# allegro/allRank

Hardware: NVIDIA H100
Metric: slates/sec (higher is better)
Workload: dtype tf32

## Files before the change

### allrank_b200/csrc/gemm_tf32.h

```cpp
#pragma once
#include <cstdint>
#include <cuda_runtime.h>

#include "dropout.cuh"

namespace arb {

struct TRef {
  const void* ptr = nullptr;
  int64_t dim[4] = {1, 1, 1, 1};
  int64_t stride[4] = {1, 0, 0, 0};
  int bf16 = 0;
};

enum : int {
  EPI_BIAS = 1,
  EPI_RELU = 2,
  EPI_ADD_AUX = 4,
  EPI_MASK_AUX = 8,
  EPI_ATOMIC = 16,
  EPI_DROPOUT = 32,
  EPI_COLSUM = 64,
  EPI_RELU_BITS = 128,
  EPI_MASK_BITS = 256,
};

struct GemmDesc {
  int M = 0, N = 0, K = 0;
  int a_mn = 0, b_mn = 0;
  int b_tf32 = 0;
  int dgrad = 0;
  TRef A, B, C, Aux;
  int nb2 = 1, nb3 = 1;
  int a_b2 = 0, a_b3 = 0, b_b2 = 0, b_b3 = 0, c_b2 = 0, c_b3 = 0;
  int block_n = 64;
  int split_k = 1;
  int flags = 0;
  float alpha = 1.0f;
  const float* bias = nullptr;
  float* atomic_out = nullptr;
  int64_t atomic_ld = 0;
  DropSite drop{0u, 0u, 1.0f};
  float* colsum_out = nullptr;
  uint32_t* bits = nullptr;
  const int* rows_dev = nullptr;
};

int launch_gemm_tf32(const GemmDesc& d, cudaStream_t stream);

struct TmapBox { uint32_t b[4]; };
int make_tmap_4d(void* out_CUtensorMap, const TRef& t, TmapBox box, int unswizzled);

void set_tf32_round_on_load(int enable);
int tf32_round_on_load();
void set_gemm_persistent(int on);

}
```

### allrank_b200/csrc/scorer.cu

```cuda
#include <cstdint>
#include <string>
#include <vector>
#include <cuda_runtime.h>

#include "attention_fused.h"
#include "common.h"
#include "defaults.h"
#include "gemm_tf32.h"
#include "scorer_kernels.h"

namespace arb {

static inline int64_t align_up(int64_t v, int64_t a) { return (v + a - 1) / a * a; }

static int g_attn_mode = 2;
static int g_skip_padding = ARB_DEFAULT_SKIP_PADDING;
static int g_pack_rows = ARB_DEFAULT_PACK_ROWS;
static bool use_fused(const arb_scorer_config& c, int S) {
  return g_attn_mode >= 1 && c.n_layers > 0 && attn_fused_supported(S, c.d_model / c.n_heads);
}
static bool use_fused_bwd(const arb_scorer_config& c, int S) {
  return g_attn_mode >= 2 && use_fused(c, S) && attn_fused_bwd_supported(S, c.d_model / c.n_heads);
}

static inline int n_outputs(const arb_scorer_config& c) { return c.d_output > 1 ? c.d_output : 1; }

static int g_relu_bits = ARB_DEFAULT_RELU_BITS;
static bool relu_bits(const arb_scorer_config& c) {
  return g_relu_bits && c.n_layers > 0 && !c.bf16 && c.dropout == 0.0f && c.d_ff % 32 == 0;
}

static bool pack_eligible(const arb_scorer_config& c, int S) {
  return c.n_layers > 0 && use_fused_bwd(c, S) && c.dropout == 0.0f && c.fc_dropout == 0.0f && c.pe_mode == 0 &&
         n_outputs(c) == 1;
}
static bool use_pack(const arb_scorer_config& c, int S) { return g_pack_rows && g_skip_padding && pack_eligible(c, S); }

struct ParamLayout {
  int n_fc;
  int fc_size[ARB_MAX_FC_LAYERS];
  int64_t fc_w[ARB_MAX_FC_LAYERS], fc_b[ARB_MAX_FC_LAYERS];
  int64_t in_a, in_b;
  struct Layer { int64_t wqkv, bqkv, wo, bo, w1, b1, w2, b2, ln1_a, ln1_b, ln2_a, ln2_b; };
  Layer layer[64];
  int64_t lnf_a, lnf_b, head_w, head_b, pe, total;
};

static int make_param_layout(const arb_scorer_config& c, ParamLayout& L) {
  if (c.n_layers < 0 || c.n_layers > 64) { arb_set_error("scorer: n_layers must be in [0,64]"); return ARB_E_UNSUPPORTED; }
  if (c.d_model <= 0 || c.d_model % 4 || c.n_features <= 0 || c.n_features % 4) {
    arb_set_error("scorer: d_model and (padded) n_features must be positive multiples of 4");
    return ARB_E_UNSUPPORTED;
  }
  if (c.n_layers > 0) {
    if (c.n_heads <= 0 || c.d_model % c.n_heads || (c.d_model / c.n_heads) % 4 || c.d_ff <= 0 || c.d_ff % 4) {
      arb_set_error("scorer: need d_model % h == 0, (d_model/h) % 4 == 0 and d_ff % 4 == 0");
      return ARB_E_UNSUPPORTED;
    }
    if (c.d_model / c.n_heads > 128) { arb_set_error("scorer: head width above 128 is not supported"); return ARB_E_UNSUPPORTED; }
  }
  if (c.d_model > 1024) { arb_set_error("scorer: d_model above 1024 is not supported"); return ARB_E_UNSUPPORTED; }
  if (c.bf16 && c.n_layers > 0 && (c.d_model % 8 || c.d_ff % 8 || c.d_model < 64 || c.d_ff < 64)) {
    arb_set_error("scorer: bf16 mode needs d_model and d_ff to be multiples of 8, at least 64");
    return ARB_E_UNSUPPORTED;
  }
  const int64_t d = c.d_model, F = c.n_features, f = c.d_ff;
  L.n_fc = c.n_fc_layers > 0 ? c.n_fc_layers : 1;
  if (L.n_fc > ARB_MAX_FC_LAYERS) { arb_set_error("scorer: at most 8 FC layers"); return ARB_E_UNSUPPORTED; }
  for (int i = 0; i < L.n_fc; ++i) {
    L.fc_size[i] = c.n_fc_layers > 0 ? c.fc_sizes[i] : c.d_model;
    if (L.fc_size[i] <= 0 || L.fc_size[i] % 4 || L.fc_size[i] > 8192) {
      arb_set_error("scorer: FC layer widths must be positive multiples of 4, at most 8192");
      return ARB_E_UNSUPPORTED;
    }
  }
  if (L.fc_size[L.n_fc - 1] != c.d_model) { arb_set_error("scorer: the last FC width must equal d_model"); return ARB_E_INVALID_ARG; }
  if (c.fc_act < ARB_ACT_NONE || c.fc_act > ARB_ACT_RELU) { arb_set_error("scorer: unknown FC activation"); return ARB_E_UNSUPPORTED; }
  if (c.fc_input_norm && F > 1024) { arb_set_error("scorer: input_norm supports up to 1024 features"); return ARB_E_UNSUPPORTED; }
  int64_t o = 0;
  for (int i = 0; i < L.n_fc; ++i) {
    const int64_t in = i == 0 ? F : L.fc_size[i - 1];
    L.fc_w[i] = o; o += int64_t(L.fc_size[i]) * in;
// ... 384 lines not shown
    if (!indices || !table) { arb_set_error("scorer: positional encoding needs indices and a table"); return ARB_E_INVALID_ARG; }
    ARB_TRY(pos_forward(xcur, reinterpret_cast<const long long*>(indices), mask, table, c.pe_rows, sqrtf(float(d)), k.R, d, st));
  }
  if (pack) {
    ZeroRegions z;
    for (int l = 0; l < c.n_layers; ++l) {
      if (l > 0 && !training) break;
      const auto& wl = W.layer[l];
      if (!z.add(ws + wl.ctx, bf ? d / 2 : d, bf ? d / 2 : d, 1, 0)) {
        ARB_TRY(zero_rows(z, plan, k.R, st));
        z = ZeroRegions{};
        z.add(ws + wl.ctx, bf ? d / 2 : d, bf ? d / 2 : d, 1, 0);
      }
    }
    if (z.count) ARB_TRY(zero_rows(z, plan, k.R, st));
  }
  const AttnGeom geom{B, S, h, dk, k.R, poff};
  for (int l = 0; l < c.n_layers; ++l) {
    const auto& pl = L.layer[l];
    const auto& wl = W.layer[l];
    float* xn1 = ws + wl.xn1; float* qkv = ws + wl.qkv; float* prob = ws + wl.prob; float* ctx = ws + wl.ctx;
    float* xmid = ws + wl.xmid; float* xn2 = ws + wl.xn2; float* hdn = ws + wl.hdn; float* xout = ws + wl.xout;
    ARB_TRY(ln_forward(xcur, P + pl.ln1_a, P + pl.ln1_b, c.ln_eps, k.R, d, xn1, ws + wl.mean1, ws + wl.std1, st, 0,
                       bf ? xn1 : nullptr, plan));
    ARB_TRY(linear_fwd(k, act(xn1), d, d, wt(pl.wqkv), P + pl.bqkv, 3 * d, qkv, 3 * d, 0, nullptr, 0));
    if (W.fused) {
      ARB_TRY(launch_attn_fwd(attn_fwd_args(geom, qkv, act(ctx), mask, g_skip_padding ? kext : nullptr, ws + wl.smax,
                                            ws + wl.ssum, make_drop_site(seed, l, SITE_ATTN_P, p_drop)), st));
    } else {
      {
        GemmDesc g;
        g.M = S; g.N = S; g.K = dk; g.alpha = 1.0f / sqrtf(float(dk));
        g.A = head_view(qkv, dk, S, h, B, 3 * d);
        g.B = head_view(qkv + d, dk, S, h, B, 3 * d);
        g.C = prob_view(prob, S, W.Sp, h, B);
        batch_all(g, h, B); g.block_n = 64;
        ARB_TRY(launch_gemm_tf32(g, st));
      }
      ARB_TRY(softmax_forward(prob, mask, B, h, S, W.Sp, st, make_drop_site(seed, l, SITE_ATTN_P, p_drop)));
      {
        GemmDesc g;
        g.M = S; g.N = dk; g.K = S; g.b_mn = 1;
        g.A = prob_view(prob, S, W.Sp, h, B);
        g.B = head_view(qkv + 2 * d, dk, S, h, B, 3 * d);
        g.C = head_view(ctx, dk, S, h, B, d);
        batch_all(g, h, B); g.block_n = pick_block_n(dk);
        ARB_TRY(launch_gemm_tf32(g, st));
      }
    }
    ARB_TRY(linear_fwd(k, act(ctx), d, d, wt(pl.wo), P + pl.bo, d, xmid, d, EPI_ADD_AUX, xcur, d,
                       make_drop_site(seed, l, SITE_ATTN_OUT, p_drop)));
    ARB_TRY(ln_forward(xmid, P + pl.ln2_a, P + pl.ln2_b, c.ln_eps, k.R, d, xn2, ws + wl.mean2, ws + wl.std2, st, 0,
                       bf ? xn2 : nullptr, plan));
    ARB_TRY(linear_fwd(k, act(xn2), d, d, wt(pl.w1), P + pl.b1, f, act(hdn), f, EPI_RELU, nullptr, 0,
                       make_drop_site(seed, l, SITE_FFN_HID, p_drop),
                       wl.hbits ? reinterpret_cast<uint32_t*>(ws + wl.hbits) : nullptr));
    ARB_TRY(linear_fwd(k, act(hdn), f, f, wt(pl.w2), P + pl.b2, d, xout, d, EPI_ADD_AUX, xmid, d,
                       make_drop_site(seed, l, SITE_FFN_OUT, p_drop)));
    xcur = xout;
  }
  const int has_norm = c.n_layers > 0;
  if (hidden) {
    if (has_norm)
      return ln_forward(xcur, P + L.lnf_a, P + L.lnf_b, c.ln_eps, k.R, d, hidden, ws + W.meanf, ws + W.stdf, st, 0,
                        nullptr, plan, rowmap);
    if (cudaMemcpyAsync(hidden, xcur, size_t(k.R) * d * sizeof(float), cudaMemcpyDeviceToDevice, st) != cudaSuccess) {
      arb_set_error("scorer: device copy failed"); return ARB_E_CUDA;
    }
    return ARB_OK;
  }
  if (n_outputs(c) > 1) {
    const float* xf = xcur;
    if (has_norm) {
      ARB_TRY(ln_forward(xcur, P + L.lnf_a, P + L.lnf_b, c.ln_eps, k.R, d, ws + W.xf, ws + W.meanf, ws + W.stdf, st));
      xf = ws + W.xf;
    }
    return head_multi_forward(xf, P + L.head_w, P + L.head_b, c.out_act, k.R, d, n_outputs(c), scores, st);
  }
  ARB_TRY(head_forward(xcur, has_norm ? P + L.lnf_a : nullptr, has_norm ? P + L.lnf_b : nullptr, c.ln_eps, P + L.head_w,
                       P + L.head_b, has_norm, c.out_act, k.R, d, scores, ws + W.meanf, ws + W.stdf, st, plan, rowmap));
  return ARB_OK;
}

struct ScratchLayout { int64_t dxa, dxb, dxn, dxm, dqkv, dctx, dprob, prob, delta, dfa, dfb, ext, dy16, dxin, total; };
static void make_scratch_layout(const arb_scorer_config& c, const ParamLayout& L, int B, int S, ScratchLayout& Z,
                                bool want_dx = false) {
  const int64_t R = buffer_rows(c, B, S), d = c.d_model;
  const int Sp = int(align_up(S, 4));
  int64_t o = 0;
  auto take = [&](int64_t n) { int64_t at = o; o += align_up(n, 64); return at; };
  Z.dxa = take(R * d); Z.dxb = take(R * d); Z.dxn = take(R * d);
  Z.dxm = (c.dropout > 0.0f || c.fc_dropout > 0.0f || c.pe_mode != 0) ? take(R * d) : 0;
  if (c.n_layers > 0) {
    Z.dqkv = take(R * 3 * d); Z.dctx = take(R * d);
    const bool fb = use_fused_bwd(c, S);
    Z.dprob = fb ? 0 : take(int64_t(B) * c.n_heads * S * Sp);
    Z.prob = (use_fused(c, S) && !fb) ? take(int64_t(B) * c.n_heads * S * Sp) : 0;
    Z.delta = fb ? take(int64_t(B) * c.n_heads * S) : 0;
  } else {
    Z.dqkv = Z.dctx = Z.dprob = Z.prob = Z.delta = 0;
  }
  int64_t widest = c.fc_input_norm ? c.n_features : 0;
  for (int i = 0; i + 1 < L.n_fc; ++i) widest = std::max<int64_t>(widest, L.fc_size[i]);
  if (c.fc_act != ARB_ACT_NONE) widest = std::max<int64_t>(widest, d);
  Z.dfa = widest ? take(R * widest) : 0;
  Z.dfb = widest ? take(R * widest) : 0;
  Z.ext = take(B);
  Z.dy16 = (c.bf16 && c.n_layers > 0) ? take(R * d / 2) : 0;
  Z.dxin = (want_dx && pack_eligible(c, S)) ? take(R * c.n_features) : 0;
  Z.total = o;
}
// ... 45 lines not shown
  int* gext = reinterpret_cast<int*>(scratch + Z.ext);
  const bool skip = g_skip_padding && c.n_layers > 0 && use_fused_bwd(c, S);
  const bool pack = use_pack(c, S);
  const int* plan = pack ? reinterpret_cast<const int*>(ws + W.plan) : nullptr;
  const int* rowmap = pack ? reinterpret_cast<const int*>(ws + W.rowmap) : nullptr;
  const int* poff = pack ? reinterpret_cast<const int*>(ws + W.poff) : nullptr;
  if (pack) { k.rows_dev = plan; k.R = buffer_rows(c, B, S); x = ws + W.xc; gext = reinterpret_cast<int*>(ws + W.kext); }
  else if (skip) ARB_TRY(slate_extents(mask, dhidden ? dhidden : dscores, dhidden ? d : n_outputs(c), B, S, gext, st));
  const AttnGeom geom{B, S, h, dk, k.R, poff};
  if (pack) {
    ZeroRegions z;
    z.add(dctx, d, d, 0, 256);
    z.add(dqkv, bf ? 3 * d / 2 : 3 * d, bf ? 3 * d / 2 : 3 * d, 1, 0);
    ARB_TRY(zero_rows(z, plan, k.R, st));
  }
  const int has_norm = c.n_layers > 0;
  const float* xlast = c.n_layers > 0 ? ws + W.layer[c.n_layers - 1].xout : ws + W.x0;
  float* top_bias_grad = c.n_layers > 0 ? g(L.layer[c.n_layers - 1].b2) : fc_bias_grad;
  const float* dy = top_site.thresh ? dxm : dx;
  if (dhidden) {
    if (has_norm) {
      ARB_TRY(ln_backward(dhidden, xlast, P + L.lnf_a, ws + W.meanf, ws + W.stdf, c.ln_eps, nullptr, k.R, d, dx,
                          g(L.lnf_a), g(L.lnf_b), st, dxm, top_site, top_bias_grad, 0, nullptr, dy16, plan, rowmap));
    } else if (!fc_act) {
      if (fc_site.thresh || fc_bias_grad)
        ARB_TRY(act_backward(dhidden, ws + W.x0, dx, k.R, d, ARB_ACT_NONE, fc_site, 1.0f, fc_bias_grad, st));
      dy = (fc_site.thresh || fc_bias_grad) ? dx : dhidden;
    }
  } else if (n_outputs(c) > 1) {
    if (has_norm) {
      ARB_TRY(head_multi_backward(dscores, scores, ws + W.xf, P + L.head_w, c.out_act, k.R, d, n_outputs(c), dxn,
                                  g(L.head_w), g(L.head_b), st));
      ARB_TRY(ln_backward(dxn, xlast, P + L.lnf_a, ws + W.meanf, ws + W.stdf, c.ln_eps, nullptr, k.R, d, dx,
                          g(L.lnf_a), g(L.lnf_b), st, dxm, top_site, top_bias_grad, 0, nullptr, dy16));
    } else {
      ARB_TRY(head_multi_backward(dscores, scores, xlast, P + L.head_w, c.out_act, k.R, d, n_outputs(c), dx,
                                  g(L.head_w), g(L.head_b), st, dxm, top_site, top_bias_grad));
    }
  } else {
    ARB_TRY(head_backward(dscores, scores, xlast, has_norm ? P + L.lnf_a : nullptr, has_norm ? P + L.lnf_b : nullptr,
                          ws + W.meanf, ws + W.stdf, c.ln_eps, P + L.head_w, P + L.head_b, has_norm, c.out_act, k.R, d,
                          dx, has_norm ? g(L.lnf_a) : nullptr, has_norm ? g(L.lnf_b) : nullptr, g(L.head_w),
                          g(L.head_b), st, dxm, top_site, top_bias_grad, dy16, plan, rowmap));
  }
  for (int l = c.n_layers - 1; l >= 0; --l) {
    const auto& pl = L.layer[l];
    const auto& wl = W.layer[l];
    const float* xin = (l == 0) ? ws + W.x0 : ws + W.layer[l - 1].xout;
    float* xn1 = ws + wl.xn1; float* qkv = ws + wl.qkv; float* ctx = ws + wl.ctx;
    float* prob = W.fused ? scratch + Z.prob : ws + wl.prob;
    float* xmid = ws + wl.xmid; float* xn2 = ws + wl.xn2; float* hdn = ws + wl.hdn;
    const V dyv = bf ? b16(dy16) : V(dy);
    if (G) ARB_TRY(linear_bwd_weight(k, dyv, d, d, act(hdn), f, f, G + pl.w2));
    if (wl.hbits)
      ARB_TRY(linear_bwd_input(k, dyv, d, d, wt(pl.w2), f, act(hdn), f, EPI_COLSUM, nullptr, 0, 1.0f, g(pl.b1),
                               reinterpret_cast<const uint32_t*>(ws + wl.hbits)));
    else
    ARB_TRY(linear_bwd_input(k, dyv, d, d, wt(pl.w2), f, act(hdn), f, EPI_MASK_AUX | EPI_COLSUM, act(hdn), f,
                             drop_on ? 1.0f / (1.0f - p_drop) : 1.0f, g(pl.b1)));
    if (G) ARB_TRY(linear_bwd_weight(k, act(hdn), f, f, act(xn2), d, d, G + pl.w1));
    ARB_TRY(linear_bwd_input(k, act(hdn), f, f, wt(pl.w1), d, act(dxn), d, 0, nullptr, 0));
    const DropSite site_ao = make_drop_site(seed, l, SITE_ATTN_OUT, p_drop);
    ARB_TRY(ln_backward(dxn, xmid, P + pl.ln2_a, ws + wl.mean2, ws + wl.std2, c.ln_eps, dx, k.R, d, dx_alt,
                        g(pl.ln2_a), g(pl.ln2_b), st, dxm, site_ao, g(pl.bo), 0, bf ? dxn : nullptr, dy16, plan));
    dy = site_ao.thresh ? dxm : dx_alt;
    const V dyo = bf ? b16(dy16) : V(dy);
    if (G) ARB_TRY(linear_bwd_weight(k, dyo, d, d, act(ctx), d, d, G + pl.wo));
    ARB_TRY(linear_bwd_input(k, dyo, d, d, wt(pl.wo), d, dctx, d, 0, nullptr, 0));
    if (use_fused_bwd(c, S)) {
      ARB_TRY(launch_attn_bwd(attn_bwd_args(geom, qkv, act(ctx), dctx, dqkv, mask, (skip || pack) ? gext : nullptr,
                                            ws + wl.smax, ws + wl.ssum, scratch + Z.delta, g(pl.bqkv),
                                            make_drop_site(seed, l, SITE_ATTN_P, p_drop), plan, rowmap), st));
    } else {
      const DropSite site_p = make_drop_site(seed, l, SITE_ATTN_P, p_drop);
      if (W.fused || site_p.thresh) {
        GemmDesc g;
        g.M = S; g.N = S; g.K = dk; g.alpha = alpha;
        g.A = head_view(qkv, dk, S, h, B, 3 * d);
        g.B = head_view(qkv + d, dk, S, h, B, 3 * d);
        g.C = prob_view(prob, S, W.Sp, h, B);
        batch_all(g, h, B); g.block_n = 64;
        ARB_TRY(launch_gemm_tf32(g, st));
        ARB_TRY(softmax_forward(prob, mask, B, h, S, W.Sp, st));
      }
      {
        GemmDesc g;
        g.M = S; g.N = S; g.K = dk;
        g.A = head_view(dctx, dk, S, h, B, d);
        g.B = head_view(qkv + 2 * d, dk, S, h, B, 3 * d);
        g.C = prob_view(dprob, S, W.Sp, h, B);
        batch_all(g, h, B); g.block_n = 64;
        ARB_TRY(launch_gemm_tf32(g, st));
      }
      ARB_TRY(softmax_backward(dprob, prob, int64_t(B) * h * S, S, W.Sp, st, site_p));
      {
        GemmDesc g;
        g.M = S; g.N = dk; g.K = S; g.a_mn = 1; g.b_mn = 1;
        g.A = prob_view(prob, S, W.Sp, h, B);
        g.B = head_view(dctx, dk, S, h, B, d);
        g.C = head_view(dqkv + 2 * d, dk, S, h, B, 3 * d);
        batch_all(g, h, B); g.block_n = pick_block_n(dk);
        ARB_TRY(launch_gemm_tf32(g, st));
      }
      {
        GemmDesc g;
        g.M = S; g.N = dk; g.K = S; g.b_mn = 1; g.alpha = alpha;
        g.A = prob_view(dprob, S, W.Sp, h, B);
        g.B = head_view(qkv + d, dk, S, h, B, 3 * d);
        g.C = head_view(dqkv, dk, S, h, B, 3 * d);
        batch_all(g, h, B); g.block_n = pick_block_n(dk);
        ARB_TRY(launch_gemm_tf32(g, st));
      }
      {
        GemmDesc g;
// ... 247 lines not shown
```

### include/allrank_b200.h

```cpp
#ifndef ALLRANK_B200_H
#define ALLRANK_B200_H

#include <stddef.h>
#include <stdint.h>

#ifdef __cplusplus
extern "C" {
#endif

#define ARB_OK 0
#define ARB_E_INVALID_ARG (-1)
#define ARB_E_UNSUPPORTED (-2)
#define ARB_E_CUDA (-3)
#define ARB_E_WORKSPACE (-4)

#define ARB_MAX_ATS 32

#define ARB_SCHEME_NONE 0
#define ARB_SCHEME_NDCGLOSS1 1
#define ARB_SCHEME_NDCGLOSS2 2
#define ARB_SCHEME_LAMBDARANK 3
#define ARB_SCHEME_NDCGLOSS2PP 4
#define ARB_SCHEME_RANKNET 5
#define ARB_SCHEME_RANKNET_GTDIFF 6
// ... 98 lines not shown
                               const int64_t* indices, int32_t B, int32_t S, const float* scores,
                               const float* d_scores, const float* d_hidden, float* grads, float* d_x,
                               float* workspace, int64_t workspace_floats, float* scratch, int64_t scratch_floats,
                               uint64_t seed, void* stream);

int32_t arb_scorer_forward_dseed(const arb_scorer_config* cfg, const float* params, const float* x, const uint8_t* mask,
                                 const int64_t* indices, const float* pe_table,
                                 int32_t B, int32_t S, float* scores, float* workspace, int64_t workspace_floats,
                                 int32_t training, const uint64_t* seed_dev, void* stream);
int32_t arb_scorer_encode_dseed(const arb_scorer_config* cfg, const float* params, const float* x, const uint8_t* mask,
                                const int64_t* indices, const float* pe_table,
                                int32_t B, int32_t S, float* hidden, float* workspace, int64_t workspace_floats,
                                int32_t training, const uint64_t* seed_dev, void* stream);
int32_t arb_scorer_backward_ex_dseed(const arb_scorer_config* cfg, const float* params, const float* x,
                                     const uint8_t* mask, const int64_t* indices, int32_t B, int32_t S,
                                     const float* scores, const float* d_scores, const float* d_hidden, float* grads,
                                     float* d_x, float* workspace, int64_t workspace_floats, float* scratch,
                                     int64_t scratch_floats, const uint64_t* seed_dev, void* stream);

void arb_set_attention_mode(int32_t mode);

void arb_set_attention_skip_padding(int32_t on);

void arb_set_pack_rows(int32_t on);

void arb_set_attention_bwd_persistent(int32_t on);
int32_t arb_get_pack_rows(void);

void arb_set_pdl(int32_t on);

void arb_set_attention_fwd_two_pass(int32_t on);

void arb_set_gemm_persistent(int32_t on);

void arb_set_tf32_round_on_load(int32_t enable);

int32_t arb_gemm_tf32(const float* A, const float* B, float* C, const float* aux, const float* bias, int32_t M,
                      int32_t N, int32_t K, int32_t a_mn, int32_t b_mn, int32_t batch, int64_t a_bstride,
                      int64_t b_bstride, int64_t c_bstride, int32_t block_n, int32_t flags, float alpha,
                      int32_t split_k, void* stream);

int32_t arb_gemm_bf16(const void* A, const void* B, void* C, const void* aux, const float* bias, int32_t M, int32_t N,
                      int32_t K, int32_t a_mn, int32_t b_mn, int32_t block_n, int32_t flags, float alpha,
                      int32_t split_k, int32_t out_bf16, float* colsum_out, void* stream);

int32_t arb_attention_forward(const float* qkv, const uint8_t* mask, const int32_t* extent, int32_t B, int32_t S,
                              int32_t h, int32_t dk, float p, uint64_t seed, int32_t layer, int32_t ctx_bf16,
                              void* ctx, float* stat_max, float* stat_sum, void* stream);
int32_t arb_attention_backward(const float* qkv, const void* ctx, int32_t ctx_bf16, const float* d_ctx,
                               const uint8_t* mask, const int32_t* extent, const float* stat_max,
                               const float* stat_sum, int32_t B, int32_t S, int32_t h, int32_t dk, float p,
                               uint64_t seed, int32_t layer, void* d_qkv, float* dbias_qkv, float* delta_scratch,
                               void* stream);

int32_t arb_layernorm_forward(const float* x, const float* a, const float* b, float eps, int32_t torch_mode,
                              int64_t rows, int32_t width, float* y, void* y16, float* mean, float* sd,
                              const int32_t* rows_dev, const int32_t* rowmap, void* stream);
int32_t arb_layernorm_backward(const float* dy, const void* dy16_in, const float* x, const float* a, const float* mean,
                               const float* sd, float eps, int32_t torch_mode, const float* dres, int64_t rows,
                               int32_t width, float* dx, float* grad_a, float* grad_b, float* dx_masked,
                               void* dy16_out, float* colsum_out, float p, uint64_t seed, int32_t layer, int32_t site,
                               const int32_t* rows_dev, const int32_t* rowmap, void* stream);
int32_t arb_head_forward(const float* x, const float* a, const float* b, float eps, const float* w, const float* wb,
                         int32_t has_norm, int32_t act, int64_t rows, int32_t width, float* score, float* mean,
                         float* sd, const int32_t* rows_dev, const int32_t* rowmap, void* stream);
int32_t arb_head_backward(const float* dscore, const float* score, const float* x, const float* a, const float* b,
                          const float* mean, const float* sd, float eps, const float* w, int32_t has_norm, int32_t act,
                          int64_t rows, int32_t width, float* dx, float* grad_a, float* grad_b, float* grad_w,
                          float* grad_wb, float* dx_masked, void* dy16_out, float* colsum_out, float p, uint64_t seed,
                          int32_t layer, int32_t site, const int32_t* rows_dev, const int32_t* rowmap, void* stream);
int32_t arb_head_multi_forward(const float* xf, const float* w, const float* wb, int32_t act, int64_t rows,
                               int32_t width, int32_t n, float* score, void* stream);
int32_t arb_head_multi_backward(const float* dscore, const float* score, const float* xf, const float* w, int32_t act,
                                int64_t rows, int32_t width, int32_t n, float* dxf, float* grad_w, float* grad_wb,
                                float* dx_masked, float* colsum_out, float p, uint64_t seed, int32_t layer,
                                int32_t site, void* stream);
int32_t arb_column_sums(const float* in, int64_t rows, int32_t width, int64_t ld, float* out, void* stream);
int32_t arb_softmax_forward(float* scores, const uint8_t* mask, int32_t B, int32_t h, int32_t S, int32_t pitch,
                            float p, uint64_t seed, int32_t layer, void* stream);
int32_t arb_softmax_backward(float* dprob, float* prob, int64_t rows, int32_t S, int32_t pitch, float p,
                             uint64_t seed, int32_t layer, void* stream);

int32_t arb_adam_step(float* params, const float* grads, float* exp_avg, float* exp_avg_sq, int64_t n, float lr,
                      float beta1, float beta2, float eps, float weight_decay, int32_t step, float grad_scale,
                      void* stream);
int32_t arb_adam_step_dev(float* params, const float* grads, float* exp_avg, float* exp_avg_sq, int64_t n, float lr,
                          float beta1, float beta2, float eps, float weight_decay, float* state, float grad_scale,
                          void* stream);

size_t arb_assemble_slates_smem_bytes(int32_t max_query_len, int32_t S);
int32_t arb_assemble_slates(const float* docs_x, const float* docs_y, const int64_t* offsets, int64_t n_queries,
                            const int64_t* queries, int32_t B, int32_t S, int32_t F, int32_t max_query_len,
                            uint64_t seed, float* x_out, float* y_out, int64_t* idx_out, void* stream);
int32_t arb_gather_slates(const float* x, const float* y, const int32_t* order, int32_t B, int32_t S, int32_t F,
                          float* x_out, float* y_out, void* stream);

#define ARB_CLICK_MAX_NODES 32
#define ARB_CLICK_MAX_SLATE 4096
#define ARB_CLICK_FIXED 0
#define ARB_CLICK_RANDOM 1
#define ARB_CLICK_RELEVANT 2
#define ARB_CLICK_CASCADE 3
#define ARB_CLICK_MULTIPLE 4
#define ARB_CLICK_CONDITIONED 5
#define ARB_CLICK_MAXCLICKS 6
#define ARB_CLICK_DUPLICATES 7
// ... 30 lines not shown
```

Baseline: 196,800.

## Fuse FFN two-GEMM chain into one warp-specialized WGMMA kernel for forward and backward

Adds a persistent, warp-specialized TMA/WGMMA kernel that computes relu(x·W1+b1)·W2+b2+residual per 128-row tile, keeping the hidden chunk in shared memory. The backward path applies the same chaining to the input gradient, using the stored relu bitmask and emitting the b1 column sums. The aim is to avoid writing and re-reading the full d_ff hidden activation between the two GEMMs and to save kernel launches. In training the hidden tensor is still written for weight gradients. It only engages for d_model<=128 with enough rows, and it depends on pre-transposed weight buffers (wt32/wt32t) existing in the workspace.

```diff
diff --git a/allrank_b200/csrc/ffn_chain.cu b/allrank_b200/csrc/ffn_chain.cu
--- /dev/null
+++ b/allrank_b200/csrc/ffn_chain.cu
@@ -0,0 +1,415 @@
+#include <algorithm>
+#include <cstdio>
+#include <cuda.h>
+#include <cuda_runtime.h>
+
+#include "common.h"
+#include "gemm_tf32.h"
+#include "sm90_ptx.cuh"
+
+namespace arb {
+
+namespace {
+
+constexpr int CH_ROWS = 128;
+constexpr int CH_UNITS = 64;
+constexpr int UNIT_BYTES = 64 * 128;
+constexpr int X_SLAB_BYTES = CH_ROWS * 128;
+constexpr int H_SLAB_BYTES = 64 * 128;
+constexpr int CH_THREADS = 384;
+constexpr int SMEM_LIMIT = 227 * 1024;
+
+template <int D>
+struct ChainLayout {
+  static constexpr int KB1 = D / 32;
+  static constexpr int NBU = (D + 63) / 64;
+  static constexpr int X_BYTES = KB1 * X_SLAB_BYTES;
+  static constexpr int H_BYTES = 2 * 2 * H_SLAB_BYTES;
+  static constexpr int TAIL_BYTES = 1024;
+  static constexpr int NU_FIT = (SMEM_LIMIT - 1024 - TAIL_BYTES - X_BYTES - H_BYTES) / UNIT_BYTES;
+  static constexpr int NU = NU_FIT < 16 ? NU_FIT : 16;
+  static constexpr int RING_OFF = X_BYTES + H_BYTES;
+  static constexpr int TAIL_OFF = RING_OFF + NU * UNIT_BYTES;
+  static constexpr int total() { return TAIL_OFF + TAIL_BYTES + 1024; }
+  static_assert(D % 32 == 0 && D >= 32 && D <= 256, "d: a multiple of 32 up to 256");
+  static_assert(NU >= 2 * NBU, "the ring holds at least one k-block of the second product");
+  static_assert(total() <= SMEM_LIMIT, "shared memory budget");
+};
+
+struct ChainParams {
+  int M;
+  int F;
+  int rnd;
+  int store_h;
+  const float* b1;
+  const float* b2;
+  const float* aux;
+  float* y;
+  uint32_t* bits;
+  float* colsum;
+  const int* rows_dev;
+};
+
+__device__ __forceinline__ void load_a(uint32_t (&a)[4][4], const uint8_t* slab, int r0, int rnd) {
+  const int lane = threadIdx.x & 31, j = lane >> 3;
+#pragma unroll
+  for (int ks = 0; ks < 4; ++ks) {
+    ptx::ldmatrix_x4(a[ks], slab + ptx::sw128(r0 + 8 * (j & 1) + (lane & 7), 32 * ks + 16 * (j >> 1)));
+    if (rnd) {
+#pragma unroll
+      for (int e = 0; e < 4; ++e) a[ks][e] = ptx::cvt_tf32(__uint_as_float(a[ks][e]));
+    }
+  }
+}
+
+template <int D, int U = 0>
+__device__ __forceinline__ void second_mma(float (&acc)[D / 8][4], const uint32_t (&a)[4],
+                                           const uint64_t (&desc)[(D + 63) / 64], int ks) {
+  constexpr int WN = D % 64 == 0 ? 64 : 32;
+  if constexpr (U < D / WN) {
+    if constexpr (WN == 64) ptx::wgmma_m64n64k8_tf32<8 * U>(acc, a, desc[U] + 2 * ks);
+    else ptx::wgmma_m64n32k8_tf32<4 * U>(acc, a, desc[U / 2] + (U & 1) * (32 * 128 / 16) + 2 * ks);
+    second_mma<D, U + 1>(acc, a, desc, ks);
+  }
+}
+
+template <int D, bool BWD>
+__global__ void __launch_bounds__(CH_THREADS, 1) ffn_chain_kernel(const __grid_constant__ CUtensorMap tmX,
+                                                                 const __grid_constant__ CUtensorMap tmA,
+                                                                 const __grid_constant__ CUtensorMap tmB,
+                                                                 const __grid_constant__ CUtensorMap tmH,
+                                                                 const ChainParams p) {
+  using L = ChainLayout<D>;
+  constexpr int NU = L::NU, KB1 = L::KB1, NBU = L::NBU, NTY = D / 8;
+  extern __shared__ uint8_t smem_dyn[];
+  uint8_t* smem = reinterpret_cast<uint8_t*>((reinterpret_cast<uintptr_t>(smem_dyn) + 1023) & ~uintptr_t(1023));
+  uint8_t* xs = smem;
+  uint8_t* ring = smem + L::RING_OFF;
+  uint64_t* full = reinterpret_cast<uint64_t*>(smem + L::TAIL_OFF);
+  uint64_t* empty = full + NU;
+  uint64_t* xfull = empty + NU;
+  uint64_t* xfree = xfull + 8;
+  uint64_t* csfull = xfree + 1;
+  uint64_t* csempty = csfull + 2;
+  float* csx = reinterpret_cast<float*>(smem + L::TAIL_OFF + 512);
+
+  const int warp = threadIdx.x >> 5, lane = threadIdx.x & 31;
+  if (threadIdx.x == 0) {
+    ptx::prefetch_tmap(&tmX);
+    ptx::prefetch_tmap(&tmA);
+    ptx::prefetch_tmap(&tmB);
+    if (p.store_h) ptx::prefetch_tmap(&tmH);
+    for (int s = 0; s < NU; ++s) { ptx::mbar_init(&full[s], 1); ptx::mbar_init(&empty[s], 8); }
+    for (int kb = 0; kb < KB1; ++kb) ptx::mbar_init(&xfull[kb], 1);
+    ptx::mbar_init(xfree, 8);
+    for (int b = 0; b < 2; ++b) { ptx::mbar_init(&csfull[b], 128); ptx::mbar_init(&csempty[b], 128); }
+    ptx::fence_barrier_init();
+  }
+  arb_pdl_wait();
+  __syncthreads();
+  int n_tiles = (p.M + CH_ROWS - 1) / CH_ROWS;
+  if (p.rows_dev) n_tiles = min(n_tiles, (__ldg(p.rows_dev) + CH_ROWS - 1) / CH_ROWS);
+  const int n_chunks = p.F / CH_UNITS;
+
+  if (warp >= 8) {
+    asm volatile("setmaxnreg.dec.sync.aligned.u32 40;" ::: "memory");
+    if (warp == 8 && lane == 0) {
+      uint32_t it = 0;
+      auto unit = [&](const CUtensorMap* tm, int c0, int c1) {
+        const int s = it % NU;
+        const uint32_t round = it / NU;
+        if (round > 0) ptx::mbar_wait(&empty[s], (round - 1) & 1);
+        ptx::mbar_expect_tx(&full[s], UNIT_BYTES);
+        ptx::tma_load_4d(ring + s * UNIT_BYTES, tm, &full[s], c0, c1, 0, 0);
+        ++it;
+      };
+      int local = 0;
+      for (int t = blockIdx.x; t < n_tiles; t += gridDim.x, ++local) {
+        const int m0 = t * CH_ROWS;
+        if (local > 0) ptx::mbar_wait(xfree, (local - 1) & 1);
+        for (int kb = 0; kb < KB1; ++kb) {
+          ptx::mbar_expect_tx(&xfull[kb], X_SLAB_BYTES);
+          ptx::tma_load_4d(xs + kb * X_SLAB_BYTES, &tmX, &xfull[kb], 32 * kb, m0, 0, 0);
+        }
+        if (!BWD) {
+          const long long bytes = (long long)(min(p.M, m0 + CH_ROWS) - m0) * D * 4;
+          asm volatile("cp.async.bulk.prefetch.L2.global [%0], %1;"
+                       ::"l"(p.aux + (long long)m0 * D), "r"(uint32_t(bytes)) : "memory");
+        }
+        for (int j = 0; j < n_chunks; ++j) {
+          for (int kb = 0; kb < KB1; ++kb) unit(&tmA, 32 * kb, CH_UNITS * j);
+          for (int kb2 = 0; kb2 < 2; ++kb2)
+            for (int u = 0; u < NBU; ++u) unit(&tmB, CH_UNITS * j + 32 * kb2, 64 * u);
+        }
+      }
+    }
+  } else {
+    asm volatile("setmaxnreg.inc.sync.aligned.u32 232;" ::: "memory");
+    const int g = warp >> 2, w = warp & 3, gq = lane >> 2, t4 = lane & 3, gt = threadIdx.x & 127;
+    uint8_t* hs = smem + L::X_BYTES + g * 2 * H_SLAB_BYTES;
+    const int fw = p.F >> 5;
+    uint32_t it = 0, cj = 0;
+    int local = 0;
+    for (int t = blockIdx.x; t < n_tiles; t += gridDim.x, ++local) {
+      const int m0 = t * CH_ROWS;
+      const int row0 = m0 + 64 * g + 16 * w + gq;
+      float accY[NTY][4];
+#pragma unroll
+      for (int n = 0; n < NTY; ++n) accY[n][0] = accY[n][1] = accY[n][2] = accY[n][3] = 0.f;
+#pragma unroll 1
+      for (int j = 0; j < n_chunks; ++j, ++cj) {
+        uint32_t mw[2][2] = {{0u, 0u}, {0u, 0u}};
+        if constexpr (BWD) {
+#pragma unroll
+          for (int h = 0; h < 2; ++h)
+            if (row0 + 8 * h < p.M) {
+              mw[h][0] = __ldg(p.bits + (long long)(row0 + 8 * h) * fw + 2 * j);
+              mw[h][1] = __ldg(p.bits + (long long)(row0 + 8 * h) * fw + 2 * j + 1);
+            }
+        }
+        float accH[8][4];
+#pragma unroll
+        for (int n = 0; n < 8; ++n) accH[n][0] = accH[n][1] = accH[n][2] = accH[n][3] = 0.f;
+#pragma unroll 1
+        for (int kb = 0; kb < KB1; ++kb, ++it) {
+          const int s = it % NU;
+          ptx::mbar_wait(&full[s], (it / NU) & 1);
+          if (j == 0) ptx::mbar_wait(&xfull[kb], local & 1);
+          uint32_t a[4][4];
+          load_a(a, xs + kb * X_SLAB_BYTES, 64 * g + 16 * w, p.rnd);
+          const uint64_t desc = ptx::wgmma_desc_sw128(ring + s * UNIT_BYTES);
+          ptx::wgmma_fence_acc(accH);
+          ptx::wgmma_fence();
+#pragma unroll
+          for (int ks = 0; ks < 4; ++ks) ptx::wgmma_m64n64k8_tf32<0>(accH, a[ks], desc + 2 * ks);
+          ptx::wgmma_commit();
+          ptx::wgmma_wait0();
+          ptx::wgmma_fence_acc(accH);
+          __syncwarp();
+          if (lane == 0) ptx::mbar_arrive(&empty[s]);
+        }
+        if (j == n_chunks - 1) {
+          __syncwarp();
+          if (lane == 0) ptx::mbar_arrive(xfree);
+        }
+        if (p.store_h && lane == 0) ptx::tma_store_wait_read<0>();
+        if (BWD && p.colsum) ptx::named_bar_sync(1 + g, 128);
+        __syncwarp();
+        uint32_t wb[2][2] = {{0u, 0u}, {0u, 0u}};
+#pragma unroll
+        for (int n = 0; n < 8; ++n) {
+          const int c = 8 * n + 2 * t4, bp = 8 * (n & 3) + 2 * t4;
+          float2 bb = make_float2(0.f, 0.f);
+          if constexpr (!BWD) bb = __ldg(reinterpret_cast<const float2*>(p.b1 + CH_UNITS * j + c));
+#pragma unroll
+          for (int h = 0; h < 2; ++h) {
+            float o0 = accH[n][2 * h], o1 = accH[n][2 * h + 1];
+            if constexpr (BWD) {
+              o0 = (mw[h][n >> 2] >> bp) & 1u ? o0 : 0.f;
+              o1 = (mw[h][n >> 2] >> (bp + 1)) & 1u ? o1 : 0.f;
+            } else {
+              o0 += bb.x; o1 += bb.y;
+              o0 = fmaxf(o0, 0.0f); o1 = fmaxf(o1, 0.0f);
+              wb[h][n >> 2] |= (o0 > 0.f ? 1u : 0u) << bp | (o1 > 0.f ? 1u : 0u) << (bp + 1);
+            }
+            *reinterpret_cast<float2*>(hs + (n >> 2) * H_SLAB_BYTES + ptx::sw128(16 * w + gq + 8 * h, 4 * (c & 31))) =
+                make_float2(o0, o1);
+          }
+        }
+        if (!BWD && p.bits) {
+#pragma unroll
+          for (int h = 0; h < 2; ++h)
+#pragma unroll
+            for (int s = 0; s < 2; ++s) {
+              wb[h][s] |= __shfl_xor_sync(0xffffffffu, wb[h][s], 1);
+              wb[h][s] |= __shfl_xor_sync(0xffffffffu, wb[h][s], 2);
+            }
+          const int h = t4 >> 1, s = t4 & 1;
+          const uint32_t word = t4 == 0 ? wb[0][0] : t4 == 1 ? wb[0][1] : t4 == 2 ? wb[1][0] : wb[1][1];
+          if (row0 + 8 * h < p.M) p.bits[(long long)(row0 + 8 * h) * fw + 2 * j + s] = word;
+        }
+        if (p.store_h) ptx::fence_proxy_async_smem();
+        __syncwarp();
+        if (p.store_h && lane == 0) {
+#pragma unroll
+          for (int s = 0; s < 2; ++s)
+            ptx::tma_store_4d(&tmH, hs + s * H_SLAB_BYTES + 16 * w * 128, CH_UNITS * j + 32 * s, m0 + 64 * g + 16 * w, 0, 0);
+          ptx::tma_store_commit();
+        }
+        if constexpr (BWD) {
+          if (p.colsum) {
+            ptx::named_bar_sync(1 + g, 128);
+            const int cc = gt >> 1, seg = gt & 1, c5 = cc & 31;
+            const uint8_t* slab = hs + (cc >> 5) * H_SLAB_BYTES;
+            float ts = 0.f;
+#pragma unroll 8
+            for (int r = 32 * seg; r < 32 * seg + 32; ++r)
+              ts += *reinterpret_cast<const float*>(slab + r * 128 + ((((c5 >> 2) ^ (r & 7)) << 4) | ((c5 & 3) << 2)));
+            ts += __shfl_xor_sync(0xffffffffu, ts, 1);
+            const int b = cj & 1;
+            const uint32_t use = cj >> 1;
+            if (g == 1) {
+              if (use > 0) ptx::mbar_wait(&csempty[b], (use - 1) & 1);
+              if (seg == 0) csx[b * 64 + cc] = ts;
+              ptx::mbar_arrive(&csfull[b]);
+            } else {
+              ptx::mbar_wait(&csfull[b], use & 1);
+              const float other = csx[b * 64 + cc];
+              ptx::mbar_arrive(&csempty[b]);
+              if (seg == 0) p.colsum[(long long)t * p.F + CH_UNITS * j + cc] = ts + other;
+            }
+          }
+        }
+#pragma unroll 1
+        for (int kb2 = 0; kb2 < 2; ++kb2, it += NBU) {
+          uint32_t a[4][4];
+          load_a(a, hs + kb2 * H_SLAB_BYTES, 16 * w, p.rnd);
+          uint64_t desc[NBU];
+#pragma unroll
+          for (int u = 0; u < NBU; ++u) {
+            const uint32_t iu = it + u;
+            ptx::mbar_wait(&full[iu % NU], (iu / NU) & 1);
+            desc[u] = ptx::wgmma_desc_sw128(ring + (iu % NU) * UNIT_BYTES);
+          }
+          ptx::wgmma_fence_acc(accY);
+          ptx::wgmma_fence();
+#pragma unroll
+          for (int ks = 0; ks < 4; ++ks) second_mma<D>(accY, a[ks], desc, ks);
+          ptx::wgmma_commit();
+          ptx::wgmma_wait0();
+          ptx::wgmma_fence_acc(accY);
+          __syncwarp();
+          if (lane == 0) {
+#pragma unroll
+            for (int u = 0; u < NBU; ++u) ptx::mbar_arrive(&empty[(it + u) % NU]);
+          }
+        }
+      }
+#pragma unroll
+      for (int n0 = 0; n0 < NTY; n0 += 8) {
+        constexpr int G = NTY < 8 ? NTY : 8;
+        float2 r[G][2];
+        if constexpr (!BWD) {
+#pragma unroll
+          for (int n = 0; n < G && n0 + n < NTY; ++n)
+#pragma unroll
+            for (int h = 0; h < 2; ++h)
+              r[n][h] = row0 + 8 * h < p.M
+                            ? *reinterpret_cast<const float2*>(p.aux + (long long)(row0 + 8 * h) * D + 8 * (n0 + n) + 2 * t4)
+                            : make_float2(0.f, 0.f);
+        }
+#pragma unroll
+        for (int n = 0; n < G && n0 + n < NTY; ++n) {
+          const int c = 8 * (n0 + n) + 2 * t4;
+          float2 bb = make_float2(0.f, 0.f);
+          if constexpr (!BWD) bb = __ldg(reinterpret_cast<const float2*>(p.b2 + c));
+#pragma unroll
+          for (int h = 0; h < 2; ++h) {
+            const int row = row0 + 8 * h;
+            if (row >= p.M) continue;
+            float2 o = make_float2(accY[n0 + n][2 * h], accY[n0 + n][2 * h + 1]);
+            if constexpr (!BWD) {
+              o.x += bb.x; o.y += bb.y;
+              o.x += r[n][h].x; o.y += r[n][h].y;
+            }
+            *reinterpret_cast<float2*>(p.y + (long long)row * D + c) = o;
+          }
+        }
+      }
+    }
+    if (p.store_h && lane == 0) ptx::tma_store_wait_all();
+  }
+  __syncthreads();
+}
+
+template <int D, bool BWD>
+int launch_chain_t(const CUtensorMap& tX, const CUtensorMap& tA, const CUtensorMap& tB, const CUtensorMap& tH,
+                   const ChainParams& p, int grid, cudaStream_t st) {
+  return launch(ffn_chain_kernel<D, BWD>, dim3(grid), dim3(CH_THREADS), ChainLayout<D>::total(), st, true, tX,
+                tA, tB, tH, p);
+}
+
+template <bool BWD>
+int launch_chain(int d, const CUtensorMap& tX, const CUtensorMap& tA, const CUtensorMap& tB, const CUtensorMap& tH,
+                 const ChainParams& p, int grid, cudaStream_t st) {
+  switch (d) {
+    case 32: return launch_chain_t<32, BWD>(tX, tA, tB, tH, p, grid, st);
+    case 64: return launch_chain_t<64, BWD>(tX, tA, tB, tH, p, grid, st);
+    case 96: return launch_chain_t<96, BWD>(tX, tA, tB, tH, p, grid, st);
+    case 128: return launch_chain_t<128, BWD>(tX, tA, tB, tH, p, grid, st);
+    case 160: return launch_chain_t<160, BWD>(tX, tA, tB, tH, p, grid, st);
+    case 192: return launch_chain_t<192, BWD>(tX, tA, tB, tH, p, grid, st);
+    case 224: return launch_chain_t<224, BWD>(tX, tA, tB, tH, p, grid, st);
+    case 256: return launch_chain_t<256, BWD>(tX, tA, tB, tH, p, grid, st);
+    default: arb_set_error("ffn_chain: d must be a multiple of 32 up to 256"); return ARB_E_UNSUPPORTED;
+  }
+}
+
+TRef matrix(const float* p, int64_t cols, int64_t rows) {
+  TRef t; t.ptr = p; t.dim[0] = cols; t.dim[1] = rows; t.stride[0] = 1; t.stride[1] = cols; return t;
+}
+
+}
+
+bool ffn_chain_supported(int d, int f) { return d % 32 == 0 && d >= 32 && d <= 256 && f > 0 && f % CH_UNITS == 0; }
+
+int launch_ffn_chain(const FfnChain& c, cudaStream_t st) {
+  if (!ffn_chain_supported(c.d, c.f)) {
+    arb_set_error("ffn_chain: needs d a multiple of 32 up to 256 and d_ff a multiple of 64");
+    return ARB_E_UNSUPPORTED;
+  }
+  if (c.rows < 0 || !c.x || !c.a || !c.b || !c.y || (c.bwd ? !c.bits : (!c.b1 || !c.b2 || !c.aux))) {
+    arb_set_error("ffn_chain: bad arguments");
+    return ARB_E_INVALID_ARG;
+  }
+  if (c.rows == 0) return ARB_OK;
+  alignas(64) CUtensorMap tX, tA, tB, tH;
+  int rc;
+  if ((rc = make_tmap_4d(&tX, matrix(c.x, c.d, c.rows), TmapBox{{32, CH_ROWS, 1, 1}}, 0))) return rc;
+  if ((rc = make_tmap_4d(&tA, matrix(c.a, c.d, c.f), TmapBox{{32, 64, 1, 1}}, 0))) return rc;
+  if ((rc = make_tmap_4d(&tB, matrix(c.b, c.f, c.d), TmapBox{{32, 64, 1, 1}}, 0))) return rc;
+  if (c.h) {
+    if ((rc = make_tmap_4d(&tH, matrix(c.h, c.f, c.rows), TmapBox{{32, 16, 1, 1}}, 0))) return rc;
+  } else {
+    tH = tX;
+  }
+  ChainParams p;
+  p.M = c.rows; p.F = c.f; p.rnd = tf32_round_on_load(); p.store_h = c.h != nullptr;
+  p.b1 = c.b1; p.b2 = c.b2; p.aux = c.aux; p.y = c.y; p.bits = c.bits; p.colsum = c.bwd ? c.colsum : nullptr;
+  p.rows_dev = c.rows_dev;
+  const int tiles = (c.rows + CH_ROWS - 1) / CH_ROWS;
+  const int grid = std::min(tiles, sm_count());
+  DetParts dp;
+  dp.add(p.colsum, tiles, 1, c.f, c.f);
+  if ((rc = dp.begin(st))) return rc;
+  {
+    const double R = double(c.rows) * (c.rows_dev ? arb_row_frac() : 1.0), d = c.d, f = c.f;
+    const double bytes = 4.0 * R * d * (c.bwd ? 2.0 : 3.0) + (c.h ? 4.0 * R * f : 0.0) + (c.bits ? R * f / 8.0 : 0.0);
+    char name[56];
+    std::snprintf(name, sizeof name, "ffn_chain[%s M%d d%d f%d]", c.bwd ? "bwd" : "fwd", c.rows, c.d, c.f);
+    ProfScope ps(ARB_PROF_GEMM, 4.0 * R * d * f, st, bytes, name);
+    rc = c.bwd ? launch_chain<true>(c.d, tX, tA, tB, tH, p, grid, st) : launch_chain<false>(c.d, tX, tA, tB, tH, p, grid, st);
+  }
+  if (rc) return rc;
+  return dp.finish(st);
+}
+
+}
+
+extern "C" int32_t arb_ffn_forward(const float* x, const float* w1, const float* b1, const float* w2, const float* b2,
+                                   const float* res, int32_t rows, int32_t d, int32_t d_ff, float* y, float* h,
+                                   uint32_t* bits, const int32_t* rows_dev, void* stream) {
+  arb::FfnChain c;
+  c.rows = rows; c.d = d; c.f = d_ff; c.x = x; c.a = w1; c.b = w2; c.b1 = b1; c.b2 = b2; c.aux = res;
+  c.y = y; c.h = h; c.bits = bits; c.rows_dev = rows_dev; c.bwd = 0;
+  return arb::launch_ffn_chain(c, static_cast<cudaStream_t>(stream));
+}
+
+extern "C" int32_t arb_ffn_backward_input(const float* dy, const float* w2t, const float* w1t, const uint32_t* bits,
+                                          int32_t rows, int32_t d, int32_t d_ff, float* dx, float* dh,
+                                          float* grad_b1, const int32_t* rows_dev, void* stream) {
+  arb::FfnChain c;
+  c.rows = rows; c.d = d; c.f = d_ff; c.x = dy; c.a = w2t; c.b = w1t; c.bits = const_cast<uint32_t*>(bits);
+  c.y = dx; c.h = dh; c.colsum = grad_b1; c.rows_dev = rows_dev; c.bwd = 1;
+  return arb::launch_ffn_chain(c, static_cast<cudaStream_t>(stream));
+}
diff --git a/allrank_b200/csrc/gemm_tf32.h b/allrank_b200/csrc/gemm_tf32.h
--- a/allrank_b200/csrc/gemm_tf32.h
+++ b/allrank_b200/csrc/gemm_tf32.h
@@ -48,6 +48,24 @@
 
 int launch_gemm_tf32(const GemmDesc& d, cudaStream_t stream);
 
+struct FfnChain {
+  int rows = 0, d = 0, f = 0;
+  const float* x = nullptr;
+  const float* a = nullptr;
+  const float* b = nullptr;
+  const float* b1 = nullptr;
+  const float* b2 = nullptr;
+  const float* aux = nullptr;
+  float* y = nullptr;
+  float* h = nullptr;
+  uint32_t* bits = nullptr;
+  float* colsum = nullptr;
+  const int* rows_dev = nullptr;
+  int bwd = 0;
+};
+bool ffn_chain_supported(int d, int f);
+int launch_ffn_chain(const FfnChain& c, cudaStream_t stream);
+
 struct TmapBox { uint32_t b[4]; };
 int make_tmap_4d(void* out_CUtensorMap, const TRef& t, TmapBox box, int unswizzled);
 
diff --git a/allrank_b200/csrc/scorer.cu b/allrank_b200/csrc/scorer.cu
--- a/allrank_b200/csrc/scorer.cu
+++ b/allrank_b200/csrc/scorer.cu
@@ -28,6 +28,10 @@
 static int g_relu_bits = ARB_DEFAULT_RELU_BITS;
 static bool relu_bits(const arb_scorer_config& c) {
   return g_relu_bits && c.n_layers > 0 && !c.bf16 && c.dropout == 0.0f && c.d_ff % 32 == 0;
+}
+static bool use_ffn_chain(const arb_scorer_config& c, int64_t rows) {
+  return relu_bits(c) && ffn_chain_supported(c.d_model, c.d_ff) && c.d_model <= 128 &&
+         rows >= int64_t(4) * 128 * sm_count();
 }
 
 static bool pack_eligible(const arb_scorer_config& c, int S) {
@@ -518,11 +522,21 @@
                        make_drop_site(seed, l, SITE_ATTN_OUT, p_drop)));
     ARB_TRY(ln_forward(xmid, P + pl.ln2_a, P + pl.ln2_b, c.ln_eps, k.R, d, xn2, ws + wl.mean2, ws + wl.std2, st, 0,
                        bf ? xn2 : nullptr, plan));
-    ARB_TRY(linear_fwd(k, act(xn2), d, d, wt(pl.w1), P + pl.b1, f, act(hdn), f, EPI_RELU, nullptr, 0,
-                       make_drop_site(seed, l, SITE_FFN_HID, p_drop),
-                       wl.hbits ? reinterpret_cast<uint32_t*>(ws + wl.hbits) : nullptr));
-    ARB_TRY(linear_fwd(k, act(hdn), f, f, wt(pl.w2), P + pl.b2, d, xout, d, EPI_ADD_AUX, xmid, d,
-                       make_drop_site(seed, l, SITE_FFN_OUT, p_drop)));
+    if (use_ffn_chain(c, k.R)) {
+      FfnChain fc;
+      fc.rows = int(k.R); fc.d = d; fc.f = f; fc.rows_dev = k.rows_dev;
+      fc.x = xn2; fc.a = ws + W.wt32 + pl.w1; fc.b = ws + W.wt32 + pl.w2;
+      fc.b1 = P + pl.b1; fc.b2 = P + pl.b2; fc.aux = xmid; fc.y = xout;
+      fc.h = training ? hdn : nullptr;
+      fc.bits = wl.hbits ? reinterpret_cast<uint32_t*>(ws + wl.hbits) : nullptr;
+      ARB_TRY(launch_ffn_chain(fc, st));
+    } else {
+      ARB_TRY(linear_fwd(k, act(xn2), d, d, wt(pl.w1), P + pl.b1, f, act(hdn), f, EPI_RELU, nullptr, 0,
+                         make_drop_site(seed, l, SITE_FFN_HID, p_drop),
+                         wl.hbits ? reinterpret_cast<uint32_t*>(ws + wl.hbits) : nullptr));
+      ARB_TRY(linear_fwd(k, act(hdn), f, f, wt(pl.w2), P + pl.b2, d, xout, d, EPI_ADD_AUX, xmid, d,
+                         make_drop_site(seed, l, SITE_FFN_OUT, p_drop)));
+    }
     xcur = xout;
   }
   const int has_norm = c.n_layers > 0;
@@ -674,14 +688,24 @@
     float* xmid = ws + wl.xmid; float* xn2 = ws + wl.xn2; float* hdn = ws + wl.hdn;
     const V dyv = bf ? b16(dy16) : V(dy);
     if (G) ARB_TRY(linear_bwd_weight(k, dyv, d, d, act(hdn), f, f, G + pl.w2));
-    if (wl.hbits)
-      ARB_TRY(linear_bwd_input(k, dyv, d, d, wt(pl.w2), f, act(hdn), f, EPI_COLSUM, nullptr, 0, 1.0f, g(pl.b1),
-                               reinterpret_cast<const uint32_t*>(ws + wl.hbits)));
-    else
-    ARB_TRY(linear_bwd_input(k, dyv, d, d, wt(pl.w2), f, act(hdn), f, EPI_MASK_AUX | EPI_COLSUM, act(hdn), f,
-                             drop_on ? 1.0f / (1.0f - p_drop) : 1.0f, g(pl.b1)));
-    if (G) ARB_TRY(linear_bwd_weight(k, act(hdn), f, f, act(xn2), d, d, G + pl.w1));
-    ARB_TRY(linear_bwd_input(k, act(hdn), f, f, wt(pl.w1), d, act(dxn), d, 0, nullptr, 0));
+    if (use_ffn_chain(c, k.R)) {
+      FfnChain fc;
+      fc.rows = int(k.R); fc.d = d; fc.f = f; fc.rows_dev = k.rows_dev; fc.bwd = 1;
+      fc.x = dy; fc.a = ws + W.wt32t + pl.w2; fc.b = ws + W.wt32t + pl.w1;
+      fc.bits = reinterpret_cast<uint32_t*>(ws + wl.hbits);
+      fc.h = hdn; fc.colsum = g(pl.b1); fc.y = dxn;
+      ARB_TRY(launch_ffn_chain(fc, st));
+      if (G) ARB_TRY(linear_bwd_weight(k, act(hdn), f, f, act(xn2), d, d, G + pl.w1));
+    } else {
+      if (wl.hbits)
+        ARB_TRY(linear_bwd_input(k, dyv, d, d, wt(pl.w2), f, act(hdn), f, EPI_COLSUM, nullptr, 0, 1.0f, g(pl.b1),
+                                 reinterpret_cast<const uint32_t*>(ws + wl.hbits)));
+      else
+        ARB_TRY(linear_bwd_input(k, dyv, d, d, wt(pl.w2), f, act(hdn), f, EPI_MASK_AUX | EPI_COLSUM, act(hdn), f,
+                                 drop_on ? 1.0f / (1.0f - p_drop) : 1.0f, g(pl.b1)));
+      if (G) ARB_TRY(linear_bwd_weight(k, act(hdn), f, f, act(xn2), d, d, G + pl.w1));
+      ARB_TRY(linear_bwd_input(k, act(hdn), f, f, wt(pl.w1), d, act(dxn), d, 0, nullptr, 0));
+    }
     const DropSite site_ao = make_drop_site(seed, l, SITE_ATTN_OUT, p_drop);
     ARB_TRY(ln_backward(dxn, xmid, P + pl.ln2_a, ws + wl.mean2, ws + wl.std2, c.ln_eps, dx, k.R, d, dx_alt,
                         g(pl.ln2_a), g(pl.ln2_b), st, dxm, site_ao, g(pl.bo), 0, bf ? dxn : nullptr, dy16, plan));
diff --git a/include/allrank_b200.h b/include/allrank_b200.h
--- a/include/allrank_b200.h
+++ b/include/allrank_b200.h
@@ -174,6 +174,13 @@
                                const float* stat_sum, int32_t B, int32_t S, int32_t h, int32_t dk, float p,
                                uint64_t seed, int32_t layer, void* d_qkv, float* dbias_qkv, float* delta_scratch,
                                void* stream);
+
+int32_t arb_ffn_forward(const float* x, const float* w1, const float* b1, const float* w2, const float* b2,
+                        const float* res, int32_t rows, int32_t d, int32_t d_ff, float* y, float* h, uint32_t* bits,
+                        const int32_t* rows_dev, void* stream);
+int32_t arb_ffn_backward_input(const float* dy, const float* w2t, const float* w1t, const uint32_t* bits,
+                               int32_t rows, int32_t d, int32_t d_ff, float* dx, float* dh, float* grad_b1,
+                               const int32_t* rows_dev, void* stream);
 
 int32_t arb_layernorm_forward(const float* x, const float* a, const float* b, float eps, int32_t torch_mode,
                               int64_t rows, int32_t width, float* y, void* y16, float* mean, float* sd,
```

New measurement: 208,300 (median of 6 runs). +5.8%, better.
